# OpenNLPLab/ACR_WSSS

Measured on AMD Instinct MI355X. Metric: img/s ACR-ViT-hybrid-base 448x448 train step, higher is better.
Workload: dtype f32_split; 1 GPU; BASELINE configs[1]: ViT-hybrid-base (DPT) 448x448, batch 16 per GPU, ACR train step (2 views, fwd+bwd+SGD); global_batch=16, classes=20, alpha=125, parallelism=dp1

## Files before the change

### acr_wsss_amd/_lib.py

```python
import ctypes
import os

import torch

_HERE = os.path.dirname(os.path.abspath(__file__))
LIB_PATH = os.environ.get("ACR_LIB_PATH") or os.path.join(_HERE, "libacr_hip.so")

ACR_F32, ACR_BF16, ACR_BF16_F32MATH, ACR_F32_BF16X3 = 0, 1, 2, 3
MATH = {"f32": 0, "f32_split": 1, "f32_fp16x2": 2}
BF16_F32MATH = False
GETAM_FUNCS = {"grad": 0, "cam_grad": 1, "grad_s": 2, "cam_grad_s": 3}

c_void_p, c_int32, c_int64, c_float, c_size_t = (ctypes.c_void_p, ctypes.c_int32, ctypes.c_int64,
                                                  ctypes.c_float, ctypes.c_size_t)


class AttnDesc(ctypes.Structure):
    _fields_ = [("B", c_int32), ("H", c_int32), ("T", c_int32), ("head_dim", c_int32),
                ("dtype", c_int32), ("scale", c_float),
                ("qkv_sb", c_int64), ("qkv_st", c_int64), ("qkv_sh", c_int64),
                ("o_sb", c_int64), ("o_st", c_int64), ("o_sh", c_int64)]


_P = ctypes.POINTER(AttnDesc)
SIGNATURES = {
    "acr_version": (c_int32, []),
    "acr_last_error": (ctypes.c_char_p, []),
    "acr_set_option": (c_int32, [c_int32, c_int32]),
    "acr_get_option": (c_int32, [c_int32]),
    "acr_attn_fwd": (c_int32, [_P, c_void_p, c_void_p, c_void_p, c_void_p, c_void_p, c_void_p, c_int64, c_int64,
                               c_void_p]),
    "acr_attn_bwd": (c_int32, [_P, c_void_p, c_void_p, c_void_p, c_void_p, c_void_p, c_void_p, c_void_p, c_int64,
                               c_int64, c_void_p, c_void_p, c_void_p, c_void_p, c_void_p]),
    "acr_attn_scores_floats": (c_int64, [_P]),
    "acr_attn_fwd_scores": (c_int32, [_P, c_void_p, c_void_p, c_void_p, c_void_p, c_void_p, c_void_p, c_void_p, c_int64, c_int64,
                                      c_void_p]),
    "acr_attn_fwd_scores_oimg": (c_int32, [_P, c_void_p, c_void_p, c_void_p, c_void_p, c_void_p, c_void_p, c_void_p, c_int64, c_int64,
                                           c_void_p, c_void_p]),
    "acr_attn_fwd_oimg_offered": (c_int32, [_P]),
    "acr_attn_bwd_scores": (c_int32, [_P, c_void_p, c_void_p, c_void_p, c_void_p, c_void_p, c_void_p, c_void_p, c_void_p, c_int64,
                                      c_int64, c_void_p, c_void_p, c_void_p, c_void_p, c_void_p]),
    "acr_attn_bwd_ws_floats": (c_int64, [_P]),
    "acr_split3_bf16": (c_int32, [c_void_p, c_int64, c_int64, c_int64, c_void_p, c_int64, c_void_p]),
    "acr_attn_probs": (c_int32, [_P, c_void_p, c_void_p, c_void_p, c_void_p, c_void_p]),
    "acr_attn_dprobs": (c_int32, [_P, c_void_p, c_void_p, c_void_p, c_void_p]),
    "acr_consistency_ws_floats": (c_size_t, [c_int32, c_int32, c_int32]),
    "acr_consistency_fwd": (c_int32, [c_void_p, c_void_p, c_int64, c_int32, c_int32, c_int32, c_int32, c_void_p,
                                      c_void_p, c_void_p]),
    "acr_consistency_bwd": (c_int32, [c_void_p, c_void_p, c_int64, c_int32, c_int32, c_int32, c_int32, c_void_p,
                                      c_void_p, c_void_p, c_int64, c_int64, c_void_p]),
    "acr_linear_bf16": (c_int32, [c_void_p, c_int64, c_void_p, c_int64, c_void_p, c_void_p, c_int64, c_void_p, c_int64,
                                  c_int32, c_int32, c_int32, c_void_p]),
    "acr_gemm_f32_ws_floats": (c_size_t, [c_int32, c_int32, c_int32, c_int32, c_int32]),
    "acr_x3_image_floats": (c_size_t, [c_int32, c_int32]),
# ... 218 lines not shown
```

### acr_wsss_amd/backbone.py

```python
import math
import os
from collections import OrderedDict

import torch
import torch.nn as nn
import torch.nn.functional as F

from . import ops


def set_math(module, math):
    from . import _lib
    code = _lib.MATH[math] if isinstance(math, str) else int(math)
    for m in module.modules():
        if hasattr(type(m), "acr_math"):
            m.acr_math = code if code != _lib.MATH["f32_fp16x2"] or isinstance(m, (Mlp, Attention)) else _lib.MATH["f32_split"]
    return module


def _same_pad(n, k, s):
    return max((math.ceil(n / s) - 1) * s + (k - 1) + 1 - n, 0)


def pad_same(x, k, s, value=0.0):
# ... 280 lines not shown
        self.scale = (dim // num_heads) ** -0.5
        self.qkv = nn.Linear(dim, dim * 3, bias=True)
        self.proj = nn.Linear(dim, dim)
        self._saved = None
        self._saved_do = None
        self._saved_gpm = None
        self._override = {}
        self.last_pm = None

    hip_linear = True
    acr_math = 0
    keep_state_in_training = False

    def forward(self, x, stack=None, layer=0, resid=None, x_image=None):
        self._override = {}
        qkv = ops.linear_or_hip(x, self.qkv, None, self.hip_linear, math=self.acr_math, x_image=x_image)
        core_math = 1 if self.acr_math == 2 else self.acr_math
        if (self.acr_math == 1 and self.hip_linear and ops.X3_IMAGES and ops.linear_f32_usable(qkv, self.proj.weight)
                and not torch.is_autocast_enabled() and ops._f32_ok(self.proj.weight, self.proj.bias, resid)):
            o, self.last_pm, oimg = ops.attention_core_oimg(qkv, self.num_heads, stack, layer, self, self.acr_math)
            return ops.linear_or_hip(o, self.proj, resid, self.hip_linear, math=self.acr_math, x_image=oimg)
        o, self.last_pm = ops.attention_core(qkv, self.num_heads, stack, layer, self, core_math)
        return ops.linear_or_hip(o, self.proj, resid, self.hip_linear, math=self.acr_math)

    def get_attn(self):
        if "attn" in self._override:
            return self._override["attn"]
        if self._saved is None:
            return None
        qkv, lse2, heads = self._saved
        return ops.attn_probs(qkv.detach(), lse2, heads)
# ... 405 lines not shown
```

### acr_wsss_amd/csrc/attn_f32.h

```cpp
#pragma once
#include <hip/hip_runtime.h>
#include <stdint.h>

struct AttnGeom {
    int B, H, T;
    float scale;
    int64_t sb, st, sh;
    int64_t osb, ost, osh;
};

void acr_attn_fwd_f32_dma(const AttnGeom& g, const float* q, const float* k, const float* v, float* o, float* lse2, float* pmean,
                          int64_t pmean_sb, int64_t pmean_st, hipStream_t st);
void acr_attn_bwd_f32_dma(const AttnGeom& g, const float* q, const float* k, const float* v, const float* o, const float* d_o,
                          const float* lse2, const float* gm, int64_t gm_sb, int64_t gm_st, float* dq, float* dk, float* dv,
                          float* delta, hipStream_t st);

void acr_attn_fwd_f32_sres(const AttnGeom& g, const float* q, const float* k, const float* v, float* o, float* lse2, float* scores,
                           float* pmean, int64_t pmean_sb, int64_t pmean_st, hipStream_t st);
void acr_attn_bwd_f32_sres(const AttnGeom& g, const float* q, const float* k, const float* v, const float* o, const float* d_o,
                           const float* lse2, const float* scores, const float* gm, int64_t gm_sb, int64_t gm_st, float* dq,
                           float* dk, float* dv, float* delta, hipStream_t st);
void acr_attn_pmean_sres(const AttnGeom& g, const float* scores, const float* lse2, float* pmean, int64_t pmean_sb, int64_t pmean_st,
                         hipStream_t st);
void acr_attn_delta_sres(const AttnGeom& g, const float* scores, const float* o, const float* d_o, const float* lse2, const float* gm,
                         int64_t gm_sb, int64_t gm_st, float* delta, hipStream_t st);

int64_t acr_attn_x3_scores_floats(const AttnGeom& g);
int64_t acr_attn_x3_bwd_ws_floats(const AttnGeom& g);
bool acr_attn_x3_fwd_uses_split_tail(int T);
void acr_attn_fwd_f32_x3(const AttnGeom& g, const float* q, const float* k, const float* v, float* o, float* lse2, float* scores,
                         float* pmean, int64_t pmean_sb, int64_t pmean_st, hipStream_t st, char* oimg = nullptr);
void acr_attn_bwd_f32_x3(const AttnGeom& g, const float* q, const float* k, const float* v, const float* o, const float* d_o,
                         const float* lse2, const float* scores, const float* gm, int64_t gm_sb, int64_t gm_st, float* dq, float* dk,
                         float* dv, float* delta_ws, hipStream_t st);
```

### acr_wsss_amd/csrc/attn_f32.hip

```cpp
#include "acr_common.h"
#include "attn_f32.h"
#include "attn_f32_scores.h"

#define LDP 68
#define TILE_FLOATS (32 * LDP)

template <typename T, int NTHREADS>
__device__ __forceinline__ void stage_tile(float* lds, const T* g, int64_t st, int row0, int Tn, int tid, float mul) {
#pragma unroll
    for (int i = 0; i < 512 / NTHREADS; ++i) {
        const int slot = tid + i * NTHREADS;
        const int row = slot >> 4, c4 = slot & 15;
        f32x4 v = acr_load4<T>(g + (int64_t)min(row0 + row, Tn - 1) * st + c4 * 4) * mul;
        const f32x4 z = {0.f, 0.f, 0.f, 0.f};
        *reinterpret_cast<f32x4*>(lds + row * LDP + c4 * 4) = (row0 + row < Tn) ? v : z;
    }
}

template <typename T>
__device__ __forceinline__ void load_rows(float (&reg)[32], const T* g, int64_t st, int row0, int Tn, int lane, float mul) {
    const int r = lane & 31, h = lane >> 5;
    const float okm = (row0 + r < Tn) ? mul : 0.f;
    const T* p = g + (int64_t)min(row0 + r, Tn - 1) * st + 32 * h;
#pragma unroll
// ... 606 lines not shown
    if (d->dtype != ACR_F32_BF16X3) {
        acr_set_error("acr_attn_fwd_scores_oimg: ACR_F32_BF16X3 only (the image is the split-product operand form)");
        return ACR_ERR_UNSUPPORTED;
    }
    rc = check_fwd_scores(d, "acr_attn_fwd_scores_oimg", q, k, v, o, lse2, scores, pmean, pmean_sb, pmean_st, true, o_image);
    if (rc) return rc;
    ACR_CHECK_ARG(d->o_sh == 64 && d->o_st == (int64_t)d->H * 64 && d->o_sb == (int64_t)d->T * d->o_st,
                  "acr_attn_fwd_scores_oimg: o must be the dense (B, T, H*64) activation (its image is that of the (B*T) x (H*64) matrix)");
    rc = check_x3(d, "acr_attn_fwd_scores_oimg");
    if (rc) return rc;
    acr_attn_fwd_f32_x3(geom(d), (const float*)q, (const float*)k, (const float*)v, (float*)o, lse2, scores, pmean, pmean_sb, pmean_st,
                        (hipStream_t)stream, reinterpret_cast<char*>(o_image));
    return acr_check_launch("acr_attn_fwd_scores_oimg");
}

extern "C" int acr_attn_fwd_oimg_offered(const acr_attn_desc* d) {
    if (!d || d->dtype != ACR_F32_BF16X3 || d->T <= 0) return 0;
    return acr_attn_x3_fwd_uses_split_tail(d->T) ? 0 : 1;
}

extern "C" int acr_attn_bwd_scores(const acr_attn_desc* d, const void* q, const void* k, const void* v, const void* o,
                                   const void* d_o, const float* lse2, const float* scores, const float* gmean, int64_t gmean_sb,
                                   int64_t gmean_st, void* dq, void* dk, void* dv, float* delta_ws, void* stream) {
    int rc = check_desc(d, "acr_attn_bwd_scores");
    if (rc) return rc;
    if (d->dtype != ACR_F32 && d->dtype != ACR_F32_BF16X3) {
        acr_set_error("acr_attn_bwd_scores: fp32 tensors only (the bf16 kernels recompute the logits)");
        return ACR_ERR_UNSUPPORTED;
    }
    ACR_CHECK_ARG(q && k && v && o && d_o && lse2 && scores && dq && dk && dv && delta_ws, "acr_attn_bwd_scores: null pointer");
// ... 98 lines not shown
```

### acr_wsss_amd/csrc/attn_f32_x3.hip

```cpp
#include <type_traits>

#include "acr_split.h"
#include "attn_f32.h"
#include "attn_f32_scores.h"
#include "attn_f32_sres_tails.h"

typedef __bf16 bf16_t;

#define X3_PLANE_B (32 * 64 * 2)
#define X3_TILE_B (3 * X3_PLANE_B)
#define X3_SLOT_B (2 * X3_TILE_B)


__device__ __forceinline__ void x3_wait_vm(int n) { attn_wait_vm<false, 9, 8, 7, 5, 4, 1>(n); }
__device__ __forceinline__ void x3_barrier(int n_younger) {
    x3_wait_vm(n_younger);
    acr_barrier_nofence();
}

struct X3Geom {
    int B, H, T, D;
    float scale;
    int64_t plane;
    int64_t osb, ost, osh;
// ... 507 lines not shown
static X3Geom x3_geom(const AttnGeom& g) {
    X3Geom x;
    x.B = g.B; x.H = g.H; x.T = g.T; x.D = g.H * 64; x.scale = g.scale;
    x.plane = (int64_t)g.B * g.T * x.D;
    x.osb = g.osb; x.ost = g.ost; x.osh = g.osh;
    x.sb = g.sb; x.st = g.st; x.sh = g.sh;
    return x;
}

bool acr_attn_x3_fwd_uses_split_tail(int T) {
    const int NB = (T + 31) / 32;
    return attn_split_tail(NB, 4) && NB >= 33;
}

void acr_attn_fwd_f32_x3(const AttnGeom& g, const float* q, const float* k, const float* v, float* o, float* lse2, float* scores,
                         float* pmean, int64_t pmean_sb, int64_t pmean_st, hipStream_t st, char* oimg) {
    const X3Geom x = x3_geom(g);
    bf16_t* planes = reinterpret_cast<bf16_t*>(scores + attn_score_floats(g.B, g.H, g.T));
    X3SplitArgs a;
    a.src[0] = q; a.src[1] = k; a.src[2] = v;
    a.sb = g.sb; a.st = g.st; a.sh = g.sh; a.dst = planes; a.plane = x.plane; a.B = g.B; a.T = g.T; a.H = g.H;
    const int64_t n8 = (int64_t)g.B * g.T * g.H * 8;
    hipLaunchKernelGGL(x3_split_kernel, dim3((unsigned)((n8 + 255) / 256), 3), dim3(256), 0, st, a);
    const int NB = (g.T + 31) / 32;
    const int ntail = (acr_attn_x3_fwd_uses_split_tail(g.T) && oimg == nullptr) ? g.B * g.H : 0;
    hipLaunchKernelGGL(attn_fwd_x3_kernel, dim3(g.B * g.H * (ntail ? NB / 4 : (NB + 3) / 4) + ntail), dim3(256), 0, st, x, (const bf16_t*)planes,
                       (const bf16_t*)(planes + 3 * x.plane), (const bf16_t*)(planes + 6 * x.plane), o, lse2, scores, q, k, v, g, ntail, oimg);
    if (pmean) acr_attn_pmean_sres(g, scores, lse2, pmean, pmean_sb, pmean_st, st);
}

void acr_attn_bwd_f32_x3(const AttnGeom& g, const float* q, const float* k, const float* v, const float* o, const float* d_o,
                         const float* lse2, const float* scores, const float* gm, int64_t gm_sb, int64_t gm_st, float* dq, float* dk,
                         float* dv, float* delta_ws, hipStream_t st) {
    const X3Geom x = x3_geom(g);
    const bf16_t* planes = reinterpret_cast<const bf16_t*>(scores + attn_score_floats(g.B, g.H, g.T));
    bf16_t* dop = reinterpret_cast<bf16_t*>(delta_ws + (((int64_t)g.B * g.H * g.T + 3) & ~(int64_t)3));
    X3SplitArgs a;
    a.src[0] = d_o; a.src[1] = a.src[2] = nullptr;
// ... 24 lines not shown
```

### acr_wsss_amd/csrc/gemm_planes.hip

```cpp
#include <math.h>

#include <mutex>
#include <type_traits>
#include <unordered_map>

#include "gemm_f32.h"


template <int FMT>
__device__ __forceinline__ f32x16 pl_mfma(bf16x8 a, bf16x8 b, f32x16 c) {
    if constexpr (FMT == 0) return __builtin_amdgcn_mfma_f32_32x32x16_bf16(a, b, c, 0, 0, 0);
    else return __builtin_amdgcn_mfma_f32_32x32x16_f16(__builtin_bit_cast(f16x8, a), __builtin_bit_cast(f16x8, b), c, 0, 0, 0);
}
template <int FMT, int M0, int M1>
__device__ __forceinline__ void pl_mfmas(f32x16 (&acc)[2][2], const bf16x8 (&a)[2][PlanesFmt<FMT>::NP], const bf16x8 (&b)[2][PlanesFmt<FMT>::NP]) {
    if constexpr (M0 < M1) {
        constexpr int NT = PlanesFmt<FMT>::NT, t = M0 / NT, k = M0 % NT;
        acc[t >> 1][t & 1] = pl_mfma<FMT>(a[t >> 1][pl_ta(FMT, k)], b[t & 1][pl_tb(FMT, k)], acc[t >> 1][t & 1]);
        pl_mfmas<FMT, M0 + 1, M1>(acc, a, b);
    }
}
template <int FMT, int M0, int M1>
__device__ __forceinline__ void pt_mfmas(f32x16 (&acc)[2][2], const bf16x4 (&al)[2][PlanesFmt<FMT>::NP], const bf16x4 (&ah)[2][PlanesFmt<FMT>::NP],
                                         const bf16x4 (&bl)[2][PlanesFmt<FMT>::NP], const bf16x4 (&bh)[2][PlanesFmt<FMT>::NP]) {
// ... 358 lines not shown
                const f32x4 x0 = *reinterpret_cast<const f32x4*>(xp), x1 = *reinterpret_cast<const f32x4*>(xp + 4);
#pragma unroll
                for (int e = 0; e < 8; ++e) v[e] *= e < 4 ? x0[e] : x1[e - 4];
            }
        } else {
#pragma unroll
            for (int e = 0; e < 8; ++e) v[e] = 0.f;
        }
        if (ACT == 6) {
#pragma unroll
            for (int e = 0; e < 8; ++e) csum[hf][e] += v[e];
        }
        x3_image_chunk_store(img, tm, tn, g.img_nkb, row_t, c8, v);
    }
    if (ACT == 6 && g.cs) x3_tile_colsum(csum, red, tid, g.cs + (int64_t)tm * g.N, n0, g.N);
}

template <int ACT, int FMT = 0>
__global__ __launch_bounds__(256, 2) void gemm_f32_planes_kernel(const GemmF32Args g) {
    constexpr int NP = PlanesFmt<FMT>::NP, NG = 4 * NP, NM = 4 * PlanesFmt<FMT>::NT;
    constexpr int STAGE_B = 2 * NP * IMG_PLANE_B;
    __shared__ __attribute__((aligned(1024))) float smem[P_SLOTS * STAGE_B / 4];
    typedef __attribute__((address_space(3))) void* lds_vp;
    typedef const __attribute__((address_space(1))) void* glb_vp;
    const int tid = threadIdx.x, lane = tid & 63;
    const int wave = __builtin_amdgcn_readfirstlane(tid >> 6);
    const int r = lane & 31, h = lane >> 5, wm = wave >> 1, wn = wave & 1;
    const int ntile = g.tiles_launch;
    const int t0 = acr_xcd_remap(blockIdx.x, ntile * g.nsplit);
    const int split = t0 / ntile, tt = g.tile0 + (t0 - split * ntile);
// ... 60 lines not shown
    int slot = 1;
    for (int st = 1; st < nst; st += 2) {
        step(st, slot, std::integral_constant<int, 1>{}, std::false_type{});
        slot = slot == 2 ? 0 : slot + 1;
        if (st + 1 < nst) {
            step(st + 1, slot, std::integral_constant<int, 0>{}, std::false_type{});
            slot = slot == 2 ? 0 : slot + 1;
        }
    }
    if (nst & 1) pl_mfmas<FMT, 0, NM>(acc, ap[0], bp[0]);
    else pl_mfmas<FMT, 0, NM>(acc, ap[1], bp[1]);
    asm volatile("s_waitcnt vmcnt(0)" ::: "memory");
    __syncthreads();
    if constexpr (FMT == 1) h2_unscale(g, acc, m0 + wm * 64, n0 + wn * 64, r, h);
    if constexpr (ACT == 5 || ACT == 6) x3_finish_image<ACT>(g, acc, smem, tm, tn, m0, n0, wm, wn, r, h, tid);
    else gemm_f32_finish<true, ACT>(g, acc, smem, split, tt, tn, m0, n0, zs, wm, wn, r, h, tid, 0.f, false);
}

#define PL_RDTR(lo, hi, alo, ahi, OFF)                                                                  \
    asm volatile("ds_read_b64_tr_b16 %0, %2 offset:%4\n\tds_read_b64_tr_b16 %1, %3 offset:%4"          \
                 : "=&v"(lo), "=&v"(hi) : "v"(alo), "v"(ahi), "i"(OFF))
template <int FMT = 0>
__global__ __launch_bounds__(256, 2) void gemm_f32_planes_tn_kernel(const GemmF32Args g) {
    constexpr int NP = PlanesFmt<FMT>::NP, NG = 4 * NP, NM = 4 * PlanesFmt<FMT>::NT;
    constexpr int STAGE_B = 2 * NP * IMG_PLANE_B;
    __shared__ __attribute__((aligned(1024))) float smem[P_SLOTS * STAGE_B / 4];
    typedef __attribute__((address_space(3))) void* lds_vp;
    typedef const __attribute__((address_space(1))) void* glb_vp;
    const int tid = threadIdx.x, lane = tid & 63;
    const int wave = __builtin_amdgcn_readfirstlane(tid >> 6);
    const int r = lane & 31, h = lane >> 5, wm = wave >> 1, wn = wave & 1;
// ... 193 lines not shown
        gemm_f32_reduce(ws, p.nsplit, (int64_t)M * N / 4, c, st);
        return acr_check_launch(FMT == 0 ? "acr_gemm_x3(TN)" : "acr_gemm_h2(TN)");
    }
    TailPlan tp = gemm_tail_plan(M, N, K, true);
    if (!ws) tp.ntail = 0;
    float* parts = (act == 4 && colsum) ? ws + (gemm_ws_base_floats(mode, M, N, K, true) + 3) / 4 * 4 : nullptr;
    g.cs = parts; g.img_nkb = (N + P_BK - 1) / P_BK;
    g.tiles_launch -= tp.ntail;
    if (g.tiles_launch > 0) {
        const dim3 grid((unsigned)g.tiles_launch);
        if (act == 0) hipLaunchKernelGGL((gemm_f32_planes_kernel<0, FMT>), grid, dim3(256), 0, st, g);
        else if (act == 1) hipLaunchKernelGGL((gemm_f32_planes_kernel<1, FMT>), grid, dim3(256), 0, st, g);
        else if (act == 2) hipLaunchKernelGGL((gemm_f32_planes_kernel<2, FMT>), grid, dim3(256), 0, st, g);
        else if constexpr (FMT == 0) {
            if (act == 3) hipLaunchKernelGGL((gemm_f32_planes_kernel<5>), grid, dim3(256), 0, st, g);
            else hipLaunchKernelGGL((gemm_f32_planes_kernel<6>), grid, dim3(256), 0, st, g);
        }
    }
    if (tp.ntail) {
        GemmF32Args gt = g;
        gt.tile0 = g.tiles_launch; gt.tiles_launch = tp.ntail; gt.nsplit = tp.nsplit; gt.kps = tp.kps; gt.k_zs = tp.kps; gt.c = ws;
        hipLaunchKernelGGL((gemm_f32_planes_kernel<4, FMT>), dim3((unsigned)(tp.ntail * tp.nsplit)), dim3(256), 0, st, gt);
        GemmF32Args ge = g;
        ge.tile0 = gt.tile0;
        if (act <= 2) gemm_f32_tail_epilogue(act, ge, ws, tp.ntail, tp.nsplit, st);
        else if (act == 3) hipLaunchKernelGGL((gemm_x3_tail_image_kernel<5>), dim3((unsigned)tp.ntail), dim3(256), 0, st, ge, (const float*)ws, tp.ntail, tp.nsplit);
        else hipLaunchKernelGGL((gemm_x3_tail_image_kernel<6>), dim3((unsigned)tp.ntail), dim3(256), 0, st, ge, (const float*)ws, tp.ntail, tp.nsplit);
    }
    if (parts) hipLaunchKernelGGL(planes_colsum_kernel, dim3((N + 15) / 16), dim3(256), 0, st, (const float*)parts, g.tiles_m, N, colsum);
    return acr_check_launch(FMT == 0 ? "acr_gemm_x3" : "acr_gemm_h2");
}
template int gemm_planes<1>(int32_t, int32_t, const float*, const float*, const float*, const float*, int64_t, float*, int64_t, float*, float*, int32_t,
                            int32_t, int32_t, float*, const int*, const int*, hipStream_t);
extern "C" int acr_gemm_x3(int32_t mode, int32_t act, const float* a_img, const float* b_img, const float* bias, const float* aux, int64_t ldaux,
                           float* c, int64_t ldc, float* c2, float* colsum, int32_t M, int32_t N, int32_t K, float* ws, void* stream) {
    ACR_CHECK_ARG(a_img && b_img && (c || act == 4), "acr_gemm_x3: null pointer");
    ACR_CHECK_ARG(M > 0 && N > 0 && K > 0, "acr_gemm_x3: empty problem (M=%d N=%d K=%d)", M, N, K);
    ACR_CHECK_ARG((mode == ACR_GEMM_NT || mode == ACR_GEMM_TN) && act >= 0 && act <= 4, "acr_gemm_x3: mode must be ACR_GEMM_NT or ACR_GEMM_TN (got %d), act 0..4 (got %d)", mode, act);
    ACR_CHECK_ARG(!colsum || act == 4, "acr_gemm_x3: colsum comes with act 4 only (the image passes give it otherwise)");
    ACR_CHECK_ARG(al16(a_img) && al16(b_img) && al16(c) && (ldc % 4) == 0 && (!bias || al16(bias)) && (!aux || (al16(aux) && (ldaux % 4) == 0)) && (!c2 || al16(c2)),
                  "acr_gemm_x3: pointers must be 16-byte aligned, pitches %% 4 == 0");
    ACR_CHECK_ARG(!ws || al16(ws), "acr_gemm_x3: ws must be 16-byte aligned");
    if (mode == ACR_GEMM_TN) {
        ACR_CHECK_ARG(act == 0 && !bias && !aux, "acr_gemm_x3: TN takes no epilogue");
        ACR_CHECK_ARG(ws, "acr_gemm_x3: TN needs the acr_gemm_x3_ws_floats workspace");
        ACR_CHECK_ARG((M % 4) == 0 && (N % 4) == 0 && ldc == N, "acr_gemm_x3: TN needs M, N %% 4 == 0 and a dense output (ldc == N)");
    } else {
        ACR_CHECK_ARG((act != 1 && act != 3 && act != 4) || c2, "acr_gemm_x3: act 1 / 3 / 4 need c2");
        ACR_CHECK_ARG((act != 2 && act != 4) || aux, "acr_gemm_x3: act 2 / 4 (GELU') need the saved derivative in aux");
        ACR_CHECK_ARG(act < 3 || ((N % 8) == 0 && (!aux || (ldaux % 4) == 0)), "acr_gemm_x3: image epilogues need N %% 8 == 0");
        ACR_CHECK_ARG(act != 4 || !colsum || ws, "acr_gemm_x3: act 4 with colsum needs ws");
    }
    return gemm_planes<0>(mode, act, a_img, b_img, bias, aux, ldaux, c, ldc, c2, colsum, M, N, K, ws, nullptr, nullptr, (hipStream_t)stream);
}

extern "C" size_t acr_h2_image_floats(int32_t rows, int32_t cols) {
    if (rows <= 0 || cols <= 0) return 0;
    return h2_floats(rows, cols);
}
extern "C" size_t acr_h2_ws_floats(int32_t rows, int32_t cols) {
    if (rows <= 0 || cols <= 0) return 0;
    return (size_t)((rows + F_BM - 1) / F_BM) * cols;
}
// ... 92 lines not shown
```

### acr_wsss_amd/ops.py

```python
import os
import torch
from torch.autograd import Function

from . import _lib as L

HEAD_DIM = 64
ATTN_F32_SCORES = True


def pad4(n):
    return (n + 3) & ~3


def _desc(B, H, T, dtype, packed_qkv=True, math=0):
    D = H * HEAD_DIM
    d = L.AttnDesc()
    d.B, d.H, d.T, d.head_dim = B, H, T, HEAD_DIM
    d.dtype = L.ACR_F32_BF16X3 if (math == 1 and dtype == torch.float32) else L.dtype_code(dtype)
    d.scale = HEAD_DIM ** -0.5
    d.qkv_sb, d.qkv_st, d.qkv_sh = T * 3 * D, 3 * D, HEAD_DIM
    d.o_sb, d.o_st, d.o_sh = T * D, D, HEAD_DIM
    return d


# ... 42 lines not shown

KERNEL_TIMER = None


def _t0(name, *dims):
    return KERNEL_TIMER.begin("%s %s" % (name, "x".join(str(int(d)) for d in dims))) if KERNEL_TIMER is not None else None


def _t1(tok):
    if tok is not None:
        KERNEL_TIMER.end(tok)

class AttnCoreFn(Function):

    @staticmethod
    def forward(ctx, qkv, heads, stack, layer, owner, math=0, want_oimg=False):
        L.require_gpu(qkv)
        ctx.set_materialize_grads(False)
        if not qkv.is_contiguous():
            qkv = qkv.contiguous()
        B, T, D3 = qkv.shape
        D = heads * HEAD_DIM
        assert D3 == 3 * D, "qkv last dim %d != 3*heads*64" % D3
        lib = L.load()
        keep_scores = ctx.needs_input_grad[0]
        ctx.math = math = int(math == 1 and ATTN_F32_SCORES and qkv.dtype == torch.float32 and (keep_scores or stack is not None))
        d = _desc(B, heads, T, qkv.dtype, math=math)
        o = torch.empty((B, T, D), dtype=qkv.dtype, device=qkv.device)
        lse2 = torch.empty((B, heads, T), dtype=torch.float32, device=qkv.device)
        pm = None
        if stack is not None:
            pm = stack.buf[:, layer]
        qp, kp, vp = _qkv_ptrs(qkv, heads)
        scores = None
        if ATTN_F32_SCORES and qkv.dtype == torch.float32 and (keep_scores or pm is not None):
            scores = torch.empty(lib.acr_attn_scores_floats(d), dtype=torch.float32, device=qkv.device)
        tok = _t0("attn_fwd" if pm is not None else "attn_fwd_nomean", B, heads, T)
        pm_sb, pm_st = (pm.stride(0), pm.stride(1)) if pm is not None else (0, 0)
        oimg = None
        if want_oimg and scores is not None and math == 1 and lib.acr_attn_fwd_oimg_offered(d):
            oimg = x3_image_empty(B * T, D, qkv.device)
        if oimg is not None:
            L.check(lib.acr_attn_fwd_scores_oimg(d, qp, kp, vp, L.ptr(o), L.ptr(lse2), L.ptr(scores), L.ptr(pm), pm_sb, pm_st, L.ptr(oimg),
                                                 L.stream_ptr()), "acr_attn_fwd_scores_oimg")
        elif scores is not None:
            L.check(lib.acr_attn_fwd_scores(d, qp, kp, vp, L.ptr(o), L.ptr(lse2), L.ptr(scores), L.ptr(pm), pm_sb, pm_st,
                                            L.stream_ptr()), "acr_attn_fwd_scores")
        else:
            L.check(lib.acr_attn_fwd(d, qp, kp, vp, L.ptr(o), L.ptr(lse2), L.ptr(pm), pm_sb, pm_st, L.stream_ptr()),
                    "acr_attn_fwd")
        _t1(tok)
        if scores is not None and keep_scores:
            ctx.save_for_backward(qkv, o, lse2, scores)
        else:
            ctx.save_for_backward(qkv, o, lse2)
        ctx.heads = heads
        keep = owner is not None and (not owner.training or getattr(owner, "keep_state_in_training", False))
# ... 37 lines not shown
        dqkv = torch.empty_like(qkv)
        delta = torch.empty(lib.acr_attn_bwd_ws_floats(d) if scores is not None else B * heads * T, dtype=torch.float32, device=qkv.device)
        qp, kp, vp = _qkv_ptrs(qkv, heads)
        dqp, dkp, dvp = _qkv_ptrs(dqkv, heads)
        tok = _t0("attn_bwd" if g_pm is not None else "attn_bwd_nomean", B, heads, T)
        if scores is not None:
            L.check(lib.acr_attn_bwd_scores(d, qp, kp, vp, L.ptr(o), L.ptr(d_o), L.ptr(lse2), L.ptr(scores), L.ptr(g_pm), gm_sb,
                                            gm_st, dqp, dkp, dvp, L.ptr(delta), L.stream_ptr()), "acr_attn_bwd_scores")
        else:
            L.check(lib.acr_attn_bwd(d, qp, kp, vp, L.ptr(o), L.ptr(d_o), L.ptr(lse2), L.ptr(g_pm), gm_sb, gm_st,
                                     dqp, dkp, dvp, L.ptr(delta), L.stream_ptr()), "acr_attn_bwd")
        _t1(tok)
        if ctx.owner is not None:
            ctx.owner._saved_do = d_o
            ctx.owner._saved_gpm = g_pm
        return dqkv, None, None, None, None, None, None


class StackAliasFn(Function):

    @staticmethod
    def forward(ctx, stack, *pms):
        ctx.n = len(pms)
        return stack.buf

    @staticmethod
    def backward(ctx, g):
        return (None,) + tuple(g[:, l] for l in range(ctx.n))


def attention_core(qkv, heads, stack=None, layer=0, owner=None, math=0):
    return AttnCoreFn.apply(qkv, heads, stack, layer, owner, math)


def attention_core_oimg(qkv, heads, stack=None, layer=0, owner=None, math=0):
    return AttnCoreFn.apply(qkv, heads, stack, layer, owner, math, True)


def attn_probs(qkv, lse2, heads):
    B, T, _ = qkv.shape
    lib = L.load()
    out = torch.empty((B, heads, T, T), dtype=torch.float32, device=qkv.device)
    qp, kp, _ = _qkv_ptrs(qkv, heads)
    L.check(lib.acr_attn_probs(_desc(B, heads, T, qkv.dtype), qp, kp, L.ptr(lse2), L.ptr(out), L.stream_ptr()),
            "acr_attn_probs")
    return out


def attn_dprobs(qkv, d_o, heads):
    B, T, _ = qkv.shape
    lib = L.load()
# ... 392 lines not shown
    return all(t is None or (t.dtype == torch.float32 and t.is_cuda and t.stride(-1) == 1 and (t.dim() == 1 or t.stride(0) % 4 == 0)
                             and t.data_ptr() % 16 == 0) for t in ts)


def linear_f32_usable(x, weight):
    K = x.shape[-1]
    N = weight.shape[0]
    return (x.is_cuda and x.dtype == torch.float32 and weight.dtype == torch.float32 and x.is_contiguous()
            and weight.is_contiguous() and K % 4 == 0 and N % 4 == 0 and K >= 32 and N >= 32 and x.numel() // K >= 1
            and _al16(x, weight))


class LinearF32Fn(Function):

    @staticmethod
    def forward(ctx, x, weight, bias, resid, owner=None, math=0, x_image=None):
        ctx.math = math
        shp = x.shape
        x2 = x.reshape(-1, shp[-1]) if x_image is None else None
        N = weight.shape[0]
        r2 = resid.reshape(-1, N) if resid is not None else None
        if r2 is not None and not r2.is_contiguous():
            r2 = r2.contiguous()
        M = x.numel() // shp[-1]
        y = torch.empty((M, N), dtype=torch.float32, device=x.device)
        ctx.images = math == 1 and X3_IMAGES and _f32_ok(x2, weight, y, r2, bias)
        assert ctx.images or x_image is None, "a LayerNorm image needs the split-product Linear behind it (ops.ln_image_usable)"
        if ctx.images:
            xi = x_image if x_image is not None else x3_image(x2)
            gemm_x3("nt", xi, weight_image(weight, owner), y, shp[-1], bias=bias, aux=r2)
            ctx.save_for_backward(xi if any(ctx.needs_input_grad[1:3]) else None, weight)
            ctx.M = M
        else:
            gemm_f32_raw("nt", x2, weight, y, bias=bias, aux=r2, math=math)
            ctx.save_for_backward(x2, weight)
        ctx.has_bias, ctx.has_resid, ctx.owner = bias is not None, resid is not None, owner
        return y.reshape(*shp[:-1], N)

    @staticmethod
    def backward(ctx, dy):
        x2, weight = ctx.saved_tensors
        N, K = weight.shape
        dy2 = dy.reshape(-1, N)
        if not dy2.is_contiguous():
            dy2 = dy2.contiguous()
        dx = dw = db = None
        want_db = ctx.has_bias and ctx.needs_input_grad[2]
        if ctx.images:
            if not _f32_ok(dy2):
                dy2 = dy2.clone()
            xi = x2
            db = torch.empty(N, dtype=torch.float32, device=dy.device) if want_db else None
            dyi = x3_image(dy2, colsum=db)
            if ctx.needs_input_grad[0]:
                dx = torch.empty((ctx.M, K), dtype=torch.float32, device=dy.device)
                gemm_x3("nt", dyi, weight_image(weight, ctx.owner, True), dx, N)
                dx = dx.reshape(*dy.shape[:-1], K)
            if ctx.needs_input_grad[1]:
                dw = torch.empty((N, K), dtype=torch.float32, device=dy.device)
                gemm_x3("tn", dyi, xi, dw, ctx.M)
            return dx, dw, db, (dy if ctx.has_resid else None), None, None, None
        if ctx.needs_input_grad[0]:
            dx = torch.empty((dy2.shape[0], K), dtype=torch.float32, device=dy.device)
            _dx_f32(dy2, weight, ctx.owner, dx, math=ctx.math)
            dx = dx.reshape(*dy.shape[:-1], K)
        if ctx.needs_input_grad[1]:
            dw = torch.empty((N, K), dtype=torch.float32, device=dy.device)
            db = torch.empty(N, dtype=torch.float32, device=dy.device) if want_db else None
            gemm_f32_raw("tn", dy2, x2, dw, colsum=db, math=ctx.math)
        elif want_db:
            db = dy2.sum(0)
        return dx, dw, db, (dy if ctx.has_resid else None), None, None, None


class MlpF32Fn(Function):

    @staticmethod
    def forward(ctx, x, w1, b1, w2, b2, resid, fc1=None, fc2=None, math=0, x_image=None):
        ctx.fc1, ctx.fc2, ctx.math = fc1, fc2, math
        shp = x.shape
        x2 = x.reshape(-1, shp[-1]) if x_image is None else None
        M = x.numel() // shp[-1]
        Hd, D = w1.shape[0], w2.shape[0]
        h = torch.empty((M, Hd), dtype=torch.float32, device=x.device)
        r2 = resid.reshape(-1, D) if resid is not None else None
        if r2 is not None and not r2.is_contiguous():
            r2 = r2.contiguous()
# ... 77 lines not shown
            _dx_f32(dh, w1, ctx.fc1, dx, math=math)
            dx = dx.reshape(*dy.shape[:-1], w1.shape[1])
        return dx, dw1, db1, dw2, db2, (dy if ctx.has_resid else None), None, None, None, None


def mlp_f32_usable(x, fc1, fc2, resid=None):
    return (linear_f32_usable(x, fc1.weight) and fc2.weight.dtype == torch.float32 and fc1.bias is not None
            and fc2.bias is not None and fc2.weight.is_contiguous() and fc2.weight.shape[0] % 4 == 0
            and _al16(fc2.weight, fc1.bias, fc2.bias, resid))


def mlp_f32(x, fc1, fc2, resid=None, math=0, x_image=None):
    return MlpF32Fn.apply(x, fc1.weight, fc1.bias, fc2.weight, fc2.bias, resid, fc1, fc2, math, x_image)


def linear_or_hip(x, lin, resid=None, use_hip=True, math=0, x_image=None):
    if x_image is not None:
        return LinearF32Fn.apply(x, lin.weight, lin.bias, resid, lin, math, x_image)
    if (use_hip and x.is_cuda and x.dtype == torch.bfloat16 and lin.weight.dtype == torch.bfloat16
            and lin.weight.shape[1] % 64 == 0 and x.is_contiguous() and _al16(x, lin.weight)):
        return LinearBf16Fn.apply(x, lin.weight, lin.bias, resid, lin)
    if (use_hip and linear_f32_usable(x, lin.weight) and not torch.is_autocast_enabled()
            and (math != 2 or _al16(lin.bias, resid))):
        return LinearF32Fn.apply(x, lin.weight, lin.bias, resid, lin, math)
    y = torch.nn.functional.linear(x, lin.weight, lin.bias)
    return y if resid is None else resid + y


class MaxPoolSameFn(Function):

    @staticmethod
    def forward(ctx, x, pt, pl, ph, pw):
        x = x.contiguous()
        N, C, H, W = x.shape
        Ho, Wo = (H + ph - 3) // 2 + 1, (W + pw - 3) // 2 + 1
        y = torch.empty((N, C, Ho, Wo), dtype=x.dtype, device=x.device)
        amax = torch.empty((N, C, Ho, Wo), dtype=torch.uint8, device=x.device)
        fn = L.load().acr_maxpool3x3s2_fwd_f32 if x.dtype == torch.float32 else L.load().acr_maxpool3x3s2_fwd_bf16
# ... 705 lines not shown
```

### include/acr_hip.h

```cpp
#ifndef ACR_HIP_H
#define ACR_HIP_H

#include <stddef.h>
#include <stdint.h>

#ifdef __cplusplus
extern "C" {
#endif

#define ACR_ABI_VERSION 2

typedef enum acr_status {
    ACR_OK = 0,
    ACR_ERR_INVALID = -1,
    ACR_ERR_LAUNCH = -2,
    ACR_ERR_UNSUPPORTED = -3
} acr_status;

typedef enum acr_dtype { ACR_F32 = 0, ACR_BF16 = 1, ACR_BF16_F32MATH = 2, ACR_F32_BF16X3 = 3 } acr_dtype;

typedef enum acr_math { ACR_MATH_F32 = 0, ACR_MATH_BF16X3 = 1, ACR_MATH_FP16X2 = 2 } acr_math;
#define ACR_FP16X2_REL 2.384185791015625e-07
#define ACR_FP16X2_FLOOR 1.8189894035458565e-12

// ... 23 lines not shown

int acr_attn_bwd(const acr_attn_desc* desc, const void* q, const void* k, const void* v,
                 const void* o, const void* d_o, const float* lse2,
                 const float* gmean, int64_t gmean_sb, int64_t gmean_st,
                 void* dq, void* dk, void* dv, float* delta_ws, void* stream);

int64_t acr_attn_scores_floats(const acr_attn_desc* desc);
int64_t acr_attn_bwd_ws_floats(const acr_attn_desc* desc);
int acr_split3_bf16(const float* x, int64_t rows, int64_t cols, int64_t ld, void* planes, int64_t plane_stride, void* stream);
int acr_attn_fwd_scores(const acr_attn_desc* desc, const void* q, const void* k, const void* v,
                        void* o, float* lse2, float* scores, float* pmean, int64_t pmean_sb, int64_t pmean_st, void* stream);
int acr_attn_fwd_scores_oimg(const acr_attn_desc* desc, const void* q, const void* k, const void* v,
                             void* o, float* lse2, float* scores, float* pmean, int64_t pmean_sb, int64_t pmean_st, float* o_image,
                             void* stream);
int acr_attn_fwd_oimg_offered(const acr_attn_desc* desc);
int acr_attn_bwd_scores(const acr_attn_desc* desc, const void* q, const void* k, const void* v,
                        const void* o, const void* d_o, const float* lse2, const float* scores,
                        const float* gmean, int64_t gmean_sb, int64_t gmean_st,
                        void* dq, void* dk, void* dv, float* delta_ws, void* stream);

int acr_attn_probs(const acr_attn_desc* desc, const void* q, const void* k, const float* lse2,
                   float* probs, void* stream);
int acr_attn_dprobs(const acr_attn_desc* desc, const void* d_o, const void* v,
                    float* dprobs, void* stream);

int acr_linear_bf16(const void* a, int64_t lda, const void* b, int64_t ldb, const void* bias,
                    const void* resid, int64_t ldr, void* y, int64_t ldy, int32_t M, int32_t N, int32_t K,
                    void* stream);
int acr_linear_gelu_bf16(const void* a, int64_t lda, const void* w, int64_t ldw, const void* bias, void* h, void* act,
                         int64_t ldy, int32_t M, int32_t N, int32_t K, void* stream);
// ... 262 lines not shown
```

Measured before the change: 126.2 img/s.

## Emit bf16x3 q/k/v split planes from the QKV GEMM epilogue into attention workspace

The QKV projection GEMM gains an epilogue (act 5) that also writes the three-way bf16 split planes of q, k and v straight into the attention scores workspace. The attention forward then skips its separate x3_split pass when those planes are handed over. This removes one kernel launch and a full read of the qkv activation per attention layer. In exchange the GEMM epilogue does extra stores and a second shared-memory pass, and the autograd wiring gets more complex (an extra output, a version check on the tensor).

```diff
diff --git a/acr_wsss_amd/_lib.py b/acr_wsss_amd/_lib.py
--- a/acr_wsss_amd/_lib.py
+++ b/acr_wsss_amd/_lib.py
@@ -38,6 +38,9 @@
     "acr_attn_fwd_scores_oimg": (c_int32, [_P, c_void_p, c_void_p, c_void_p, c_void_p, c_void_p, c_void_p, c_void_p, c_int64, c_int64,
                                            c_void_p, c_void_p]),
     "acr_attn_fwd_oimg_offered": (c_int32, [_P]),
+    "acr_attn_qkv_planes_offset": (c_int64, [_P]),
+    "acr_attn_fwd_scores_planes": (c_int32, [_P, c_void_p, c_void_p, c_void_p, c_void_p, c_void_p, c_void_p, c_void_p, c_int64, c_int64,
+                                             c_void_p, c_void_p]),
     "acr_attn_bwd_scores": (c_int32, [_P, c_void_p, c_void_p, c_void_p, c_void_p, c_void_p, c_void_p, c_void_p, c_void_p, c_int64,
                                       c_int64, c_void_p, c_void_p, c_void_p, c_void_p, c_void_p]),
     "acr_attn_bwd_ws_floats": (c_int64, [_P]),
diff --git a/acr_wsss_amd/backbone.py b/acr_wsss_amd/backbone.py
--- a/acr_wsss_amd/backbone.py
+++ b/acr_wsss_amd/backbone.py
@@ -318,7 +318,7 @@
 
     def forward(self, x, stack=None, layer=0, resid=None, x_image=None):
         self._override = {}
-        qkv = ops.linear_or_hip(x, self.qkv, None, self.hip_linear, math=self.acr_math, x_image=x_image)
+        qkv = ops.linear_or_hip(x, self.qkv, None, self.hip_linear, math=self.acr_math, x_image=x_image, qkv_heads=self.num_heads)
         core_math = 1 if self.acr_math == 2 else self.acr_math
         if (self.acr_math == 1 and self.hip_linear and ops.X3_IMAGES and ops.linear_f32_usable(qkv, self.proj.weight)
                 and not torch.is_autocast_enabled() and ops._f32_ok(self.proj.weight, self.proj.bias, resid)):
diff --git a/acr_wsss_amd/csrc/attn_f32.h b/acr_wsss_amd/csrc/attn_f32.h
--- a/acr_wsss_amd/csrc/attn_f32.h
+++ b/acr_wsss_amd/csrc/attn_f32.h
@@ -29,7 +29,7 @@
 int64_t acr_attn_x3_bwd_ws_floats(const AttnGeom& g);
 bool acr_attn_x3_fwd_uses_split_tail(int T);
 void acr_attn_fwd_f32_x3(const AttnGeom& g, const float* q, const float* k, const float* v, float* o, float* lse2, float* scores,
-                         float* pmean, int64_t pmean_sb, int64_t pmean_st, hipStream_t st, char* oimg = nullptr);
+                         float* pmean, int64_t pmean_sb, int64_t pmean_st, hipStream_t st, char* oimg = nullptr, bool have_planes = false);
 void acr_attn_bwd_f32_x3(const AttnGeom& g, const float* q, const float* k, const float* v, const float* o, const float* d_o,
                          const float* lse2, const float* scores, const float* gm, int64_t gm_sb, int64_t gm_st, float* dq, float* dk,
                          float* dv, float* delta_ws, hipStream_t st);
diff --git a/acr_wsss_amd/csrc/attn_f32.hip b/acr_wsss_amd/csrc/attn_f32.hip
--- a/acr_wsss_amd/csrc/attn_f32.hip
+++ b/acr_wsss_amd/csrc/attn_f32.hip
@@ -644,6 +644,29 @@
     return acr_check_launch("acr_attn_fwd_scores_oimg");
 }
 
+extern "C" int64_t acr_attn_qkv_planes_offset(const acr_attn_desc* d) {
+    if (d == nullptr || d->B <= 0 || d->H <= 0 || d->T <= 0 || d->dtype != ACR_F32_BF16X3) return -1;
+    return attn_score_floats(d->B, d->H, d->T);
+}
+extern "C" int acr_attn_fwd_scores_planes(const acr_attn_desc* d, const void* q, const void* k, const void* v, void* o, float* lse2,
+                                          float* scores, float* pmean, int64_t pmean_sb, int64_t pmean_st, float* o_image, void* stream) {
+    int rc = check_desc(d, "acr_attn_fwd_scores_planes");
+    if (rc) return rc;
+    if (d->dtype != ACR_F32_BF16X3) {
+        acr_set_error("acr_attn_fwd_scores_planes: ACR_F32_BF16X3 only (the planes are the split-product operand form)");
+        return ACR_ERR_UNSUPPORTED;
+    }
+    rc = check_fwd_scores(d, "acr_attn_fwd_scores_planes", q, k, v, o, lse2, scores, pmean, pmean_sb, pmean_st, o_image != nullptr, o_image);
+    if (rc) return rc;
+    ACR_CHECK_ARG(!o_image || (d->o_sh == 64 && d->o_st == (int64_t)d->H * 64 && d->o_sb == (int64_t)d->T * d->o_st),
+                  "acr_attn_fwd_scores_planes: o must be the dense (B, T, H*64) activation (its image is that of the (B*T) x (H*64) matrix)");
+    rc = check_x3(d, "acr_attn_fwd_scores_planes");
+    if (rc) return rc;
+    acr_attn_fwd_f32_x3(geom(d), (const float*)q, (const float*)k, (const float*)v, (float*)o, lse2, scores, pmean, pmean_sb, pmean_st,
+                        (hipStream_t)stream, reinterpret_cast<char*>(o_image), true);
+    return acr_check_launch("acr_attn_fwd_scores_planes");
+}
+
 extern "C" int acr_attn_fwd_oimg_offered(const acr_attn_desc* d) {
     if (!d || d->dtype != ACR_F32_BF16X3 || d->T <= 0) return 0;
     return acr_attn_x3_fwd_uses_split_tail(d->T) ? 0 : 1;
diff --git a/acr_wsss_amd/csrc/attn_f32_x3.hip b/acr_wsss_amd/csrc/attn_f32_x3.hip
--- a/acr_wsss_amd/csrc/attn_f32_x3.hip
+++ b/acr_wsss_amd/csrc/attn_f32_x3.hip
@@ -545,14 +545,16 @@
 }
 
 void acr_attn_fwd_f32_x3(const AttnGeom& g, const float* q, const float* k, const float* v, float* o, float* lse2, float* scores,
-                         float* pmean, int64_t pmean_sb, int64_t pmean_st, hipStream_t st, char* oimg) {
+                         float* pmean, int64_t pmean_sb, int64_t pmean_st, hipStream_t st, char* oimg, bool have_planes) {
     const X3Geom x = x3_geom(g);
     bf16_t* planes = reinterpret_cast<bf16_t*>(scores + attn_score_floats(g.B, g.H, g.T));
-    X3SplitArgs a;
-    a.src[0] = q; a.src[1] = k; a.src[2] = v;
-    a.sb = g.sb; a.st = g.st; a.sh = g.sh; a.dst = planes; a.plane = x.plane; a.B = g.B; a.T = g.T; a.H = g.H;
-    const int64_t n8 = (int64_t)g.B * g.T * g.H * 8;
-    hipLaunchKernelGGL(x3_split_kernel, dim3((unsigned)((n8 + 255) / 256), 3), dim3(256), 0, st, a);
+    if (!have_planes) {
+        X3SplitArgs a;
+        a.src[0] = q; a.src[1] = k; a.src[2] = v;
+        a.sb = g.sb; a.st = g.st; a.sh = g.sh; a.dst = planes; a.plane = x.plane; a.B = g.B; a.T = g.T; a.H = g.H;
+        const int64_t n8 = (int64_t)g.B * g.T * g.H * 8;
+        hipLaunchKernelGGL(x3_split_kernel, dim3((unsigned)((n8 + 255) / 256), 3), dim3(256), 0, st, a);
+    }
     const int NB = (g.T + 31) / 32;
     const int ntail = (acr_attn_x3_fwd_uses_split_tail(g.T) && oimg == nullptr) ? g.B * g.H : 0;
     hipLaunchKernelGGL(attn_fwd_x3_kernel, dim3(g.B * g.H * (ntail ? NB / 4 : (NB + 3) / 4) + ntail), dim3(256), 0, st, x, (const bf16_t*)planes,
diff --git a/acr_wsss_amd/csrc/gemm_planes.hip b/acr_wsss_amd/csrc/gemm_planes.hip
--- a/acr_wsss_amd/csrc/gemm_planes.hip
+++ b/acr_wsss_amd/csrc/gemm_planes.hip
@@ -396,6 +396,68 @@
         x3_image_chunk_store(img, tm, tn, g.img_nkb, row_t, c8, v);
     }
     if (ACT == 6 && g.cs) x3_tile_colsum(csum, red, tid, g.cs + (int64_t)tm * g.N, n0, g.N);
+}
+
+__device__ __forceinline__ void x3_qkv_chunk_store(const GemmF32Args& g, int row, int col, const float (&v)[8]) {
+    const int D = g.N / 3, w = col / D;
+    const int64_t plane = (int64_t)g.M * D;
+    bf16x8 p0, p1, p2;
+    split3_bf16(v, p0, p1, p2);
+    __bf16* dst = reinterpret_cast<__bf16*>(g.c2) + (int64_t)(3 * w) * plane + (int64_t)row * D + (col - w * D);
+    *reinterpret_cast<bf16x8*>(dst) = p0;
+    *reinterpret_cast<bf16x8*>(dst + plane) = p1;
+    *reinterpret_cast<bf16x8*>(dst + 2 * plane) = p2;
+}
+__device__ __forceinline__ void x3_finish_qkv_planes(const GemmF32Args& g, f32x16 (&acc)[2][2], float* tl, int m0, int n0, int wm, int wn, int r,
+                                                     int h, int tid) {
+#pragma unroll
+    for (int j = 0; j < 2; ++j) {
+        const int col_t = wn * 64 + j * 32 + r, col = n0 + col_t;
+        const float bj = (g.bias && col < g.N) ? g.bias[col] : 0.f;
+#pragma unroll
+        for (int i = 0; i < 2; ++i)
+#pragma unroll
+            for (int e = 0; e < 16; ++e) tl[(wm * 64 + i * 32 + acr_krow(e, h)) * X3E_PITCH + col_t] = acc[i][j][e] + bj;
+    }
+    __syncthreads();
+#pragma unroll
+    for (int hf = 0; hf < 2; ++hf)
+#pragma unroll
+        for (int j = 0; j < 4; ++j) {
+            const int row_t = j * 32 + (tid >> 3), c8 = hf * 8 + (tid & 7);
+            const int row = m0 + row_t, col = n0 + c8 * 8;
+            if (row >= g.M || col >= g.N) continue;
+            const f32x4 a = *reinterpret_cast<const f32x4*>(tl + row_t * X3E_PITCH + c8 * 8);
+            const f32x4 b = *reinterpret_cast<const f32x4*>(tl + row_t * X3E_PITCH + c8 * 8 + 4);
+            const float v[8] = {a[0], a[1], a[2], a[3], b[0], b[1], b[2], b[3]};
+            x3_qkv_chunk_store(g, row, col, v);
+        }
+}
+__global__ __launch_bounds__(256) void gemm_x3_tail_qkv_kernel(const GemmF32Args g, const float* __restrict__ ws, int ntail, int nsplit) {
+    const int tid = threadIdx.x, tix = blockIdx.x;
+    int tm, tn;
+    tile_coords(g.tile0 + tix, g.tiles_m, g.tiles_n, tm, tn);
+#pragma unroll
+    for (int hj = 0; hj < 8; ++hj) {
+        const int row_t = (hj & 3) * 32 + (tid >> 3), c8 = (hj >> 2) * 8 + (tid & 7);
+        const int row = tm * F_BM + row_t, col = tn * F_BN + c8 * 8;
+        if (row >= g.M || col >= g.N) continue;
+        const float* p = ws + (int64_t)tix * (F_BM * F_BN) + row_t * F_BN + c8 * 8;
+        f32x4 a = *reinterpret_cast<const f32x4*>(p), b = *reinterpret_cast<const f32x4*>(p + 4);
+        for (int k = 1; k < nsplit; ++k) {
+            const float* q = p + (int64_t)k * ntail * (F_BM * F_BN);
+            const f32x4 u = *reinterpret_cast<const f32x4*>(q), w = *reinterpret_cast<const f32x4*>(q + 4);
+            a[0] += u[0]; a[1] += u[1]; a[2] += u[2]; a[3] += u[3]; b[0] += w[0]; b[1] += w[1]; b[2] += w[2]; b[3] += w[3];
+        }
+        if (g.bias) {
+            const f32x4 u = *reinterpret_cast<const f32x4*>(g.bias + col), w = *reinterpret_cast<const f32x4*>(g.bias + col + 4);
+            a[0] += u[0]; a[1] += u[1]; a[2] += u[2]; a[3] += u[3]; b[0] += w[0]; b[1] += w[1]; b[2] += w[2]; b[3] += w[3];
+        }
+        float* cp = g.c + (int64_t)row * g.ldc + col;
+        *reinterpret_cast<f32x4*>(cp) = a; *reinterpret_cast<f32x4*>(cp + 4) = b;
+        const float v[8] = {a[0], a[1], a[2], a[3], b[0], b[1], b[2], b[3]};
+        x3_qkv_chunk_store(g, row, col, v);
+    }
 }
 
 template <int ACT, int FMT = 0>
@@ -486,7 +548,10 @@
     __syncthreads();
     if constexpr (FMT == 1) h2_unscale(g, acc, m0 + wm * 64, n0 + wn * 64, r, h);
     if constexpr (ACT == 5 || ACT == 6) x3_finish_image<ACT>(g, acc, smem, tm, tn, m0, n0, wm, wn, r, h, tid);
-    else gemm_f32_finish<true, ACT>(g, acc, smem, split, tt, tn, m0, n0, zs, wm, wn, r, h, tid, 0.f, false);
+    else if constexpr (ACT == 7) {
+        gemm_f32_finish<true, 0>(g, acc, smem, split, tt, tn, m0, n0, zs, wm, wn, r, h, tid, 0.f, false);
+        x3_finish_qkv_planes(g, acc, smem, m0, n0, wm, wn, r, h, tid);
+    } else gemm_f32_finish<true, ACT>(g, acc, smem, split, tt, tn, m0, n0, zs, wm, wn, r, h, tid, 0.f, false);
 }
 
 #define PL_RDTR(lo, hi, alo, ahi, OFF)                                                                  \
@@ -710,6 +775,7 @@
         else if (act == 2) hipLaunchKernelGGL((gemm_f32_planes_kernel<2, FMT>), grid, dim3(256), 0, st, g);
         else if constexpr (FMT == 0) {
             if (act == 3) hipLaunchKernelGGL((gemm_f32_planes_kernel<5>), grid, dim3(256), 0, st, g);
+            else if (act == 5) hipLaunchKernelGGL((gemm_f32_planes_kernel<7>), grid, dim3(256), 0, st, g);
             else hipLaunchKernelGGL((gemm_f32_planes_kernel<6>), grid, dim3(256), 0, st, g);
         }
     }
@@ -721,6 +787,7 @@
         ge.tile0 = gt.tile0;
         if (act <= 2) gemm_f32_tail_epilogue(act, ge, ws, tp.ntail, tp.nsplit, st);
         else if (act == 3) hipLaunchKernelGGL((gemm_x3_tail_image_kernel<5>), dim3((unsigned)tp.ntail), dim3(256), 0, st, ge, (const float*)ws, tp.ntail, tp.nsplit);
+        else if (act == 5) hipLaunchKernelGGL(gemm_x3_tail_qkv_kernel, dim3((unsigned)tp.ntail), dim3(256), 0, st, ge, (const float*)ws, tp.ntail, tp.nsplit);
         else hipLaunchKernelGGL((gemm_x3_tail_image_kernel<6>), dim3((unsigned)tp.ntail), dim3(256), 0, st, ge, (const float*)ws, tp.ntail, tp.nsplit);
     }
     if (parts) hipLaunchKernelGGL(planes_colsum_kernel, dim3((N + 15) / 16), dim3(256), 0, st, (const float*)parts, g.tiles_m, N, colsum);
@@ -732,7 +799,7 @@
                            float* c, int64_t ldc, float* c2, float* colsum, int32_t M, int32_t N, int32_t K, float* ws, void* stream) {
     ACR_CHECK_ARG(a_img && b_img && (c || act == 4), "acr_gemm_x3: null pointer");
     ACR_CHECK_ARG(M > 0 && N > 0 && K > 0, "acr_gemm_x3: empty problem (M=%d N=%d K=%d)", M, N, K);
-    ACR_CHECK_ARG((mode == ACR_GEMM_NT || mode == ACR_GEMM_TN) && act >= 0 && act <= 4, "acr_gemm_x3: mode must be ACR_GEMM_NT or ACR_GEMM_TN (got %d), act 0..4 (got %d)", mode, act);
+    ACR_CHECK_ARG((mode == ACR_GEMM_NT || mode == ACR_GEMM_TN) && act >= 0 && act <= 5, "acr_gemm_x3: mode must be ACR_GEMM_NT or ACR_GEMM_TN (got %d), act 0..5 (got %d)", mode, act);
     ACR_CHECK_ARG(!colsum || act == 4, "acr_gemm_x3: colsum comes with act 4 only (the image passes give it otherwise)");
     ACR_CHECK_ARG(al16(a_img) && al16(b_img) && al16(c) && (ldc % 4) == 0 && (!bias || al16(bias)) && (!aux || (al16(aux) && (ldaux % 4) == 0)) && (!c2 || al16(c2)),
                   "acr_gemm_x3: pointers must be 16-byte aligned, pitches %% 4 == 0");
@@ -742,7 +809,8 @@
         ACR_CHECK_ARG(ws, "acr_gemm_x3: TN needs the acr_gemm_x3_ws_floats workspace");
         ACR_CHECK_ARG((M % 4) == 0 && (N % 4) == 0 && ldc == N, "acr_gemm_x3: TN needs M, N %% 4 == 0 and a dense output (ldc == N)");
     } else {
-        ACR_CHECK_ARG((act != 1 && act != 3 && act != 4) || c2, "acr_gemm_x3: act 1 / 3 / 4 need c2");
+        ACR_CHECK_ARG((act != 1 && act != 3 && act != 4 && act != 5) || c2, "acr_gemm_x3: act 1 / 3 / 4 / 5 need c2");
+        ACR_CHECK_ARG(act != 5 || (!aux && (N % 24) == 0), "acr_gemm_x3: act 5 (q/k/v planes) takes no aux and needs N = 3 D with D %% 8 == 0");
         ACR_CHECK_ARG((act != 2 && act != 4) || aux, "acr_gemm_x3: act 2 / 4 (GELU') need the saved derivative in aux");
         ACR_CHECK_ARG(act < 3 || ((N % 8) == 0 && (!aux || (ldaux % 4) == 0)), "acr_gemm_x3: image epilogues need N %% 8 == 0");
         ACR_CHECK_ARG(act != 4 || !colsum || ws, "acr_gemm_x3: act 4 with colsum needs ws");
diff --git a/acr_wsss_amd/ops.py b/acr_wsss_amd/ops.py
--- a/acr_wsss_amd/ops.py
+++ b/acr_wsss_amd/ops.py
@@ -80,11 +80,11 @@
 class AttnCoreFn(Function):
 
     @staticmethod
-    def forward(ctx, qkv, heads, stack, layer, owner, math=0, want_oimg=False):
+    def forward(ctx, qkv, heads, stack, layer, owner, math=0, want_oimg=False, qkv_scores=None):
         L.require_gpu(qkv)
         ctx.set_materialize_grads(False)
         if not qkv.is_contiguous():
-            qkv = qkv.contiguous()
+            qkv, qkv_scores = qkv.contiguous(), None
         B, T, D3 = qkv.shape
         D = heads * HEAD_DIM
         assert D3 == 3 * D, "qkv last dim %d != 3*heads*64" % D3
@@ -99,14 +99,23 @@
             pm = stack.buf[:, layer]
         qp, kp, vp = _qkv_ptrs(qkv, heads)
         scores = None
+        ctx.qkv_planes_given = False
         if ATTN_F32_SCORES and qkv.dtype == torch.float32 and (keep_scores or pm is not None):
-            scores = torch.empty(lib.acr_attn_scores_floats(d), dtype=torch.float32, device=qkv.device)
+            n = lib.acr_attn_scores_floats(d)
+            if (qkv_scores is not None and math == 1 and qkv_scores.numel() == n and qkv_scores.device == qkv.device
+                    and qkv_scores.dtype == torch.float32 and qkv_scores.is_contiguous()):
+                scores, ctx.qkv_planes_given = qkv_scores, True
+            else:
+                scores = torch.empty(n, dtype=torch.float32, device=qkv.device)
         tok = _t0("attn_fwd" if pm is not None else "attn_fwd_nomean", B, heads, T)
         pm_sb, pm_st = (pm.stride(0), pm.stride(1)) if pm is not None else (0, 0)
         oimg = None
         if want_oimg and scores is not None and math == 1 and lib.acr_attn_fwd_oimg_offered(d):
             oimg = x3_image_empty(B * T, D, qkv.device)
-        if oimg is not None:
+        if ctx.qkv_planes_given:
+            L.check(lib.acr_attn_fwd_scores_planes(d, qp, kp, vp, L.ptr(o), L.ptr(lse2), L.ptr(scores), L.ptr(pm), pm_sb, pm_st, L.ptr(oimg),
+                                                   L.stream_ptr()), "acr_attn_fwd_scores_planes")
+        elif oimg is not None:
             L.check(lib.acr_attn_fwd_scores_oimg(d, qp, kp, vp, L.ptr(o), L.ptr(lse2), L.ptr(scores), L.ptr(pm), pm_sb, pm_st, L.ptr(oimg),
                                                  L.stream_ptr()), "acr_attn_fwd_scores_oimg")
         elif scores is not None:
@@ -174,7 +183,7 @@
         if ctx.owner is not None:
             ctx.owner._saved_do = d_o
             ctx.owner._saved_gpm = g_pm
-        return dqkv, None, None, None, None, None, None
+        return dqkv, None, None, None, None, None, None, None
 
 
 class StackAliasFn(Function):
@@ -189,12 +198,22 @@
         return (None,) + tuple(g[:, l] for l in range(ctx.n))
 
 
+QKV_PLANES = True
+
+
+def _qkv_scores(qkv, heads):
+    g = getattr(qkv, "_acr_qkv_scores", None)
+    if g is None or not QKV_PLANES or g[1] != heads or g[2] != qkv._version:
+        return None
+    return g[0]
+
+
 def attention_core(qkv, heads, stack=None, layer=0, owner=None, math=0):
-    return AttnCoreFn.apply(qkv, heads, stack, layer, owner, math)
+    return AttnCoreFn.apply(qkv, heads, stack, layer, owner, math, False, _qkv_scores(qkv, heads))
 
 
 def attention_core_oimg(qkv, heads, stack=None, layer=0, owner=None, math=0):
-    return AttnCoreFn.apply(qkv, heads, stack, layer, owner, math, True)
+    return AttnCoreFn.apply(qkv, heads, stack, layer, owner, math, True, _qkv_scores(qkv, heads))
 
 
 def attn_probs(qkv, lse2, heads):
@@ -617,7 +636,8 @@
 class LinearF32Fn(Function):
 
     @staticmethod
-    def forward(ctx, x, weight, bias, resid, owner=None, math=0, x_image=None):
+    def forward(ctx, x, weight, bias, resid, owner=None, math=0, x_image=None, qkv_heads=0):
+        ctx.set_materialize_grads(not qkv_heads)
         ctx.math = math
         shp = x.shape
         x2 = x.reshape(-1, shp[-1]) if x_image is None else None
@@ -631,19 +651,34 @@
         assert ctx.images or x_image is None, "a LayerNorm image needs the split-product Linear behind it (ops.ln_image_usable)"
         if ctx.images:
             xi = x_image if x_image is not None else x3_image(x2)
-            gemm_x3("nt", xi, weight_image(weight, owner), y, shp[-1], bias=bias, aux=r2)
+            scores = None
+            if (qkv_heads and QKV_PLANES and ATTN_F32_SCORES and len(shp) == 3 and N == 3 * qkv_heads * HEAD_DIM and r2 is None
+                    and any(ctx.needs_input_grad[:3])):
+                lib = L.load()
+                d = _desc(shp[0], qkv_heads, shp[1], torch.float32, math=1)
+                scores = torch.empty(lib.acr_attn_scores_floats(d), dtype=torch.float32, device=x.device)
+                gemm_x3("nt", xi, weight_image(weight, owner), y, shp[-1], bias=bias, act=5, c2=scores[lib.acr_attn_qkv_planes_offset(d):])
+                ctx.mark_non_differentiable(scores)
+            else:
+                gemm_x3("nt", xi, weight_image(weight, owner), y, shp[-1], bias=bias, aux=r2)
             ctx.save_for_backward(xi if any(ctx.needs_input_grad[1:3]) else None, weight)
             ctx.M = M
         else:
+            scores = None
             gemm_f32_raw("nt", x2, weight, y, bias=bias, aux=r2, math=math)
             ctx.save_for_backward(x2, weight)
         ctx.has_bias, ctx.has_resid, ctx.owner = bias is not None, resid is not None, owner
+        ctx.qkv_planes = scores is not None
+        if qkv_heads:
+            return y.reshape(*shp[:-1], N), scores
         return y.reshape(*shp[:-1], N)
 
     @staticmethod
-    def backward(ctx, dy):
+    def backward(ctx, dy, *unused):
         x2, weight = ctx.saved_tensors
         N, K = weight.shape
+        if dy is None:
+            return (None,) * 8
         dy2 = dy.reshape(-1, N)
         if not dy2.is_contiguous():
             dy2 = dy2.contiguous()
@@ -662,7 +697,7 @@
             if ctx.needs_input_grad[1]:
                 dw = torch.empty((N, K), dtype=torch.float32, device=dy.device)
                 gemm_x3("tn", dyi, xi, dw, ctx.M)
-            return dx, dw, db, (dy if ctx.has_resid else None), None, None, None
+            return dx, dw, db, (dy if ctx.has_resid else None), None, None, None, None
         if ctx.needs_input_grad[0]:
             dx = torch.empty((dy2.shape[0], K), dtype=torch.float32, device=dy.device)
             _dx_f32(dy2, weight, ctx.owner, dx, math=ctx.math)
@@ -673,7 +708,7 @@
             gemm_f32_raw("tn", dy2, x2, dw, colsum=db, math=ctx.math)
         elif want_db:
             db = dy2.sum(0)
-        return dx, dw, db, (dy if ctx.has_resid else None), None, None, None
+        return dx, dw, db, (dy if ctx.has_resid else None), None, None, None, None
 
 
 class MlpF32Fn(Function):
@@ -781,14 +816,26 @@
     return MlpF32Fn.apply(x, fc1.weight, fc1.bias, fc2.weight, fc2.bias, resid, fc1, fc2, math, x_image)
 
 
-def linear_or_hip(x, lin, resid=None, use_hip=True, math=0, x_image=None):
+def _linear_f32_qkv(x, lin, math, x_image, qkv_heads):
+    y, scores = LinearF32Fn.apply(x, lin.weight, lin.bias, None, lin, math, x_image, qkv_heads)
+    if scores is not None:
+        y._acr_qkv_scores = (scores, qkv_heads, y._version)
+    return y
+
+
+def linear_or_hip(x, lin, resid=None, use_hip=True, math=0, x_image=None, qkv_heads=0):
+    qkv_heads = qkv_heads if (math == 1 and resid is None and QKV_PLANES and X3_IMAGES and torch.is_grad_enabled() and lin.training) else 0
     if x_image is not None:
+        if qkv_heads:
+            return _linear_f32_qkv(x, lin, math, x_image, qkv_heads)
         return LinearF32Fn.apply(x, lin.weight, lin.bias, resid, lin, math, x_image)
     if (use_hip and x.is_cuda and x.dtype == torch.bfloat16 and lin.weight.dtype == torch.bfloat16
             and lin.weight.shape[1] % 64 == 0 and x.is_contiguous() and _al16(x, lin.weight)):
         return LinearBf16Fn.apply(x, lin.weight, lin.bias, resid, lin)
     if (use_hip and linear_f32_usable(x, lin.weight) and not torch.is_autocast_enabled()
             and (math != 2 or _al16(lin.bias, resid))):
+        if qkv_heads:
+            return _linear_f32_qkv(x, lin, math, None, qkv_heads)
         return LinearF32Fn.apply(x, lin.weight, lin.bias, resid, lin, math)
     y = torch.nn.functional.linear(x, lin.weight, lin.bias)
     return y if resid is None else resid + y
diff --git a/include/acr_hip.h b/include/acr_hip.h
--- a/include/acr_hip.h
+++ b/include/acr_hip.h
@@ -61,6 +61,10 @@
                              void* o, float* lse2, float* scores, float* pmean, int64_t pmean_sb, int64_t pmean_st, float* o_image,
                              void* stream);
 int acr_attn_fwd_oimg_offered(const acr_attn_desc* desc);
+int64_t acr_attn_qkv_planes_offset(const acr_attn_desc* desc);
+int acr_attn_fwd_scores_planes(const acr_attn_desc* desc, const void* q, const void* k, const void* v,
+                               void* o, float* lse2, float* scores, float* pmean, int64_t pmean_sb, int64_t pmean_st, float* o_image,
+                               void* stream);
 int acr_attn_bwd_scores(const acr_attn_desc* desc, const void* q, const void* k, const void* v,
                         const void* o, const void* d_o, const float* lse2, const float* scores,
                         const float* gmean, int64_t gmean_sb, int64_t gmean_st,
```

Result: no change. 126.8 img/s, median of 6 (+0.4%).
